# 0xPARC/plonkathon

Measured on NVIDIA H100. Metric: plonk_proofs_per_s_2^20_gates, higher is better.
Workload: dtype u256 (BN254 Fr/Fq integers, 8x32-bit Montgomery limbs)

## Files before the change

### include/plonk_b200.h

```cpp
#ifndef PLONK_B200_H
#define PLONK_B200_H
#include <stddef.h>
#include <stdint.h>

#ifdef __cplusplus
extern "C" {
#endif

typedef struct pb200_ctx pb200_ctx;
typedef struct pb200_srs pb200_srs;
typedef struct pb200_prover pb200_prover;
typedef struct pb200_transcript pb200_transcript;

const char* pb200_last_error(void);
const char* pb200_version(void);
int pb200_ctx_create(int device, void* cuda_stream, pb200_ctx** out);
void pb200_ctx_destroy(pb200_ctx* ctx);
int pb200_ctx_sync(pb200_ctx* ctx);
uint64_t pb200_ctx_launches(pb200_ctx* ctx);
int pb200_ctx_timing(pb200_ctx* ctx, int enable);
int pb200_ctx_timing_read(pb200_ctx* ctx, int category, double* total_ms, uint64_t* count);
void* pb200_ctx_stream(pb200_ctx* ctx);

int pb200_fr_to_mont(pb200_ctx* ctx, const void* d_in, void* d_out, uint64_t n);
// ... 5 lines not shown
int pb200_fr_ntt(pb200_ctx* ctx, const void* d_in, void* d_out, unsigned log_n, int inverse);
int pb200_fr_ntt_host(pb200_ctx* ctx, const uint8_t* h_in, uint8_t* h_out, unsigned log_n, int inverse);

int pb200_fr_ntt_decimated(pb200_ctx* ctx, const void* d_in, void* d_out, unsigned log_m, int inverse, uint64_t stride,
                           uint64_t offset);

int pb200_fr_coset_extend(pb200_ctx* ctx, const void* d_in, void* d_out, unsigned log_n, const uint8_t* h_offset);
int pb200_fr_coset_extend_host(pb200_ctx* ctx, const uint8_t* h_in, uint8_t* h_out, unsigned log_n,
                               const uint8_t* h_offset);
int pb200_fr_coset_to_coeffs(pb200_ctx* ctx, const void* d_in, void* d_out, unsigned log_n, const uint8_t* h_offset);
int pb200_fr_coset_to_coeffs_host(pb200_ctx* ctx, const uint8_t* h_in, uint8_t* h_out, unsigned log_n,
                                  const uint8_t* h_offset);
int pb200_fr_barycentric_eval(pb200_ctx* ctx, const void* d_vals, unsigned log_n, const uint8_t* h_x, uint8_t* h_out);
int pb200_fr_barycentric_eval_host(pb200_ctx* ctx, const uint8_t* h_vals, unsigned log_n, const uint8_t* h_x,
                                   uint8_t* h_out);

int pb200_g1_msm(pb200_ctx* ctx, const void* d_points, const void* d_scalars, uint64_t n, uint8_t* h_out_xy,
                 int* is_identity);
int pb200_g1_msm_host(pb200_ctx* ctx, const uint8_t* h_points, const uint8_t* h_scalars, uint64_t n,
                      uint8_t* h_out_xy, int* is_identity);

int pb200_srs_create(pb200_ctx* ctx, const uint8_t* h_points, uint64_t n, int precompute, pb200_srs** out);
int pb200_srs_generate(pb200_ctx* ctx, const uint8_t* h_tau, uint64_t n, int precompute, pb200_srs** out);
int pb200_srs_generate_lagrange(pb200_ctx* ctx, const uint8_t* h_tau, uint64_t n, int precompute, pb200_srs** out);
int pb200_srs_export(pb200_ctx* ctx, pb200_srs* srs, uint8_t* h_points, uint64_t first, uint64_t count);
void pb200_srs_destroy(pb200_srs* srs);
uint64_t pb200_srs_size(pb200_srs* srs);
int pb200_srs_commit_lagrange(pb200_ctx* ctx, pb200_srs* srs, const void* d_values, unsigned log_n,
                              uint8_t* h_out_xy, int* is_identity);
int pb200_srs_commit_lagrange_host(pb200_ctx* ctx, pb200_srs* srs, const uint8_t* h_values, unsigned log_n,
                                   uint8_t* h_out_xy, int* is_identity);
int pb200_srs_commit_coeffs(pb200_ctx* ctx, pb200_srs* srs, const void* d_coeffs, uint64_t m, int coeffs_montgomery,
                            uint8_t* h_out_xy, int* is_identity);
int pb200_srs_commit_coeffs_host(pb200_ctx* ctx, pb200_srs* srs, const uint8_t* h_coeffs, uint64_t m,
                                 uint8_t* h_out_xy, int* is_identity);

int pb200_prover_create(pb200_ctx* ctx, pb200_srs* srs, unsigned log_n, const uint8_t* const* h_pk,
                        pb200_prover** out);
int pb200_prover_create_custom(pb200_ctx* ctx, pb200_srs* srs, unsigned log_n, const uint8_t* const* h_pk,
                               unsigned n_custom, const uint8_t* h_exps, const uint8_t* const* h_custom,
                               pb200_prover** out);
void pb200_prover_destroy(pb200_prover* p);
int pb200_prover_prove(pb200_prover* p, const uint8_t* h_A, const uint8_t* h_B, const uint8_t* h_C,
                       const uint8_t* h_public, uint64_t n_public, uint8_t* h_proof768);
int pb200_prover_prove_device(pb200_prover* p, const void* d_A, const void* d_B, const void* d_C,
                              const uint8_t* h_public, uint64_t n_public, uint8_t* h_proof768);
int pb200_prover_round1(pb200_prover* p, const uint8_t* h_A, const uint8_t* h_B, const uint8_t* h_C,
                        const uint8_t* h_public, uint64_t n_public, uint8_t* h_abc_xy );
int pb200_prover_round2(pb200_prover* p, const uint8_t* beta, const uint8_t* gamma, uint8_t* h_z_xy);
int pb200_prover_round3(pb200_prover* p, const uint8_t* alpha, const uint8_t* fft_cofactor,
                        uint8_t* h_t_xy );
int pb200_prover_round4(pb200_prover* p, const uint8_t* zeta, uint8_t* h_evals );
int pb200_prover_round5(pb200_prover* p, const uint8_t* v, uint8_t* h_w_xy );

int pb200_prover_read_vector(pb200_prover* p, int which, void* d_out);
int pb200_prover_set_zk(pb200_prover* p, int enable, const uint8_t* h_blinders);
int pb200_prover_serialize(pb200_prover* p, uint8_t* h_proof768);

int pb200_prover_set_lookup(pb200_prover* p, const uint8_t* h_qk, const uint8_t* h_t1, const uint8_t* h_t2,
                            const uint8_t* h_t3, uint64_t table_rows);
int pb200_prover_set_lookup_tagged(pb200_prover* p, const uint8_t* h_qk, const uint8_t* h_qtag, const uint8_t* h_t1,
                                   const uint8_t* h_t2, const uint8_t* h_t3, const uint8_t* h_t4, uint64_t table_rows);
int pb200_prover_round_lookup(pb200_prover* p, const uint8_t* eta, uint8_t* h_fh_xy );
int pb200_prover_round2_lookup(pb200_prover* p, const uint8_t* beta, const uint8_t* gamma, const uint8_t* delta,
                               const uint8_t* epsilon, uint8_t* h_zz2_xy );
int pb200_prover_round4_lookup(pb200_prover* p, const uint8_t* zeta, uint8_t* h_evals );
// ... 65 lines not shown
```

### plonkathon_b200/_lib.py

```python
from __future__ import annotations

import ctypes
import os
import threading

_HERE = os.path.dirname(os.path.abspath(__file__))
LIB_PATH = os.environ.get("PB200_LIB") or os.path.join(_HERE, "libplonk_b200.so")

c_u8p = ctypes.POINTER(ctypes.c_uint8)


class PlonkB200Error(RuntimeError):
    pass


def _load():
    if not os.path.exists(LIB_PATH):
        raise PlonkB200Error(
            "libplonk_b200.so is not built (%s); run `python -c 'import __graft_entry__ as g; g.build()'`"
            % LIB_PATH)
    lib = ctypes.CDLL(LIB_PATH)
    V, I, U, U64 = ctypes.c_void_p, ctypes.c_int, ctypes.c_uint, ctypes.c_uint64
    P = ctypes.POINTER
    sig = {
# ... 10 lines not shown
        "pb200_fr_from_mont": (I, [V, V, V, U64]),
        "pb200_fr_ntt": (I, [V, V, V, U, I]),
        "pb200_fr_ntt_host": (I, [V, V, V, U, I]),
        "pb200_fr_ntt_decimated": (I, [V, V, V, U, I, U64, U64]),
        "pb200_fr_ntt_sharded": (I, [V, V, V, U, I]),
        "pb200_fr_vec_op": (I, [V, I, V, V, V, V, U64, U64]),
        "pb200_prover_read_vector": (I, [V, I, V]),
        "pb200_comm_unique_id": (I, [V]),
        "pb200_comm_init": (I, [V, V, I, I]),
        "pb200_comm_info": (I, [V, P(I), P(I), P(U64), P(U64)]),
        "pb200_srs_commit_coeffs_sharded": (I, [V, V, V, U64, I, V, P(I)]),
        "pb200_prover_create_sharded": (I, [V, V, U, V, P(V)]),
        "pb200_srs_commit_partial": (I, [V, V, V, U64, U64, U, U, I, V]),
        "pb200_srs_bucket_count": (I, [V, P(U)]),
        "pb200_g1_join_bucket_shards_host": (I, [V, U, U, U, V, P(I)]),
        "pb200_fr_coset_extend": (I, [V, V, V, U, V]),
        "pb200_fr_coset_extend_host": (I, [V, V, V, U, V]),
        "pb200_fr_coset_to_coeffs": (I, [V, V, V, U, V]),
        "pb200_fr_coset_to_coeffs_host": (I, [V, V, V, U, V]),
        "pb200_fr_barycentric_eval": (I, [V, V, U, V, V]),
        "pb200_fr_barycentric_eval_host": (I, [V, V, U, V, V]),
        "pb200_g1_msm": (I, [V, V, V, U64, V, P(I)]),
        "pb200_g1_msm_host": (I, [V, V, V, U64, V, P(I)]),
        "pb200_srs_create": (I, [V, V, U64, I, P(V)]),
        "pb200_srs_generate": (I, [V, V, U64, I, P(V)]),
        "pb200_srs_generate_lagrange": (I, [V, V, U64, I, P(V)]),
        "pb200_srs_export": (I, [V, V, V, U64, U64]),
        "pb200_srs_destroy": (None, [V]),
        "pb200_srs_size": (U64, [V]),
        "pb200_srs_commit_lagrange": (I, [V, V, V, U, V, P(I)]),
        "pb200_srs_commit_lagrange_host": (I, [V, V, V, U, V, P(I)]),
        "pb200_srs_commit_coeffs_host": (I, [V, V, V, U64, V, P(I)]),
        "pb200_srs_commit_coeffs": (I, [V, V, V, U64, I, V, P(I)]),
        "pb200_prover_create": (I, [V, V, U, V, P(V)]),
        "pb200_prover_create_custom": (I, [V, V, U, V, U, V, V, P(V)]),
        "pb200_prover_create_custom_sharded": (I, [V, V, U, V, U, V, V, P(V)]),
        "pb200_prover_destroy": (None, [V]),
        "pb200_prover_prove": (I, [V, V, V, V, V, U64, V]),
        "pb200_prover_prove_device": (I, [V, V, V, V, V, U64, V]),
        "pb200_prover_round1": (I, [V, V, V, V, V, U64, V]),
        "pb200_prover_round2": (I, [V, V, V, V]),
        "pb200_prover_round3": (I, [V, V, V, V]),
        "pb200_prover_round4": (I, [V, V, V]),
        "pb200_prover_round5": (I, [V, V, V]),
        "pb200_prover_serialize": (I, [V, V]),
        "pb200_prover_set_zk": (I, [V, I, V]),
        "pb200_prover_set_zk_lookup": (I, [V, I, V]),
        "pb200_prover_set_lookup": (I, [V, V, V, V, V, U64]),
        "pb200_prover_set_lookup_tagged": (I, [V, V, V, V, V, V, V, U64]),
        "pb200_prover_round_lookup": (I, [V, V, V]),
        "pb200_prover_round2_lookup": (I, [V, V, V, V, V, V]),
        "pb200_prover_round4_lookup": (I, [V, V, V]),
        "pb200_prover_prove_lookup": (I, [V, V, V, V, V, U64, V]),
        "pb200_prover_serialize_lookup": (I, [V, V]),
        "pb200_prover_create_custom_next_row": (I, [V, V, U, V, U, V, V, P(V)]),
        "pb200_prover_round4_next_row": (I, [V, V, V]),
        "pb200_prover_prove_next_row": (I, [V, V, V, V, V, U64, V]),
        "pb200_prover_serialize_next_row": (I, [V, V]),
        "pb200_prover_set_shuffle": (I, [V, V, V]),
        "pb200_prover_round2_shuffle": (I, [V, V, V, V, V, V]),
        "pb200_prover_round4_shuffle": (I, [V, V, V]),
        "pb200_prover_round4_next_row_shuffle": (I, [V, V, V]),
        "pb200_prover_prove_shuffle": (I, [V, V, V, V, V, U64, V]),
        "pb200_prover_serialize_shuffle": (I, [V, V]),
        "pb200_prover_prove_next_row_shuffle": (I, [V, V, V, V, V, U64, V]),
        "pb200_prover_serialize_next_row_shuffle": (I, [V, V]),
# ... 76 lines not shown
```

### plonkathon_b200/csrc/capi.cu

```cuda
#include "../../include/plonk_b200.h"

#include <cstring>

#include "common.cuh"
#include "comm.cuh"
#include "msm_bucket.cuh"
#include "prover.cuh"
#include "pairing.cuh"
#include "transcript.cuh"

namespace pb200 {
void ntt_run(Context* ctx, const Fr* in, Fr* out, int log_n, bool inverse, uint64_t n_in, const Fr* in_scale,
             const Fr* out_scale);
void launch_powers(Context* ctx, Fr* out, uint64_t n, const Fr& base, const Fr& scale);
Fr fr_from_u64(uint64_t x);
void ntt_run_strided(Context* ctx, const Fr* in, Fr* out, int log_n, bool inverse, uint64_t n_in,
                     const Fr* in_scale, const Fr* out_scale, uint64_t in_mul, uint64_t in_add);
void ntt_sharded(Context* ctx, const Fr* const* in, Fr* const* out, int count, int log_n, bool inverse);
void fr_to_mont(Context* ctx, const Fr* in, Fr* out, uint64_t n);
void fr_from_mont(Context* ctx, const Fr* in, Fr* out, uint64_t n);
void fr_vec_op(Context* ctx, int op, const Fr* a, const Fr* b, const Fr& scalar_canonical, Fr* out, uint64_t n,
               uint64_t shift);
void barycentric_eval(Context* ctx, const Fr* d_vals, int log_n, const Fr& x_mont, Fr* h_out);
float bench_modmul(Context* ctx, int field, uint64_t threads, uint32_t iters);
// ... 358 lines not shown
  PB_API_BEGIN PB_ON_CTX(C(ctx));
  srs_export(C(ctx), reinterpret_cast<Srs*>(srs), h_points, first, count);
  PB_API_END
}
void pb200_srs_destroy(pb200_srs* srs) { srs_destroy(reinterpret_cast<Srs*>(srs)); }
uint64_t pb200_srs_size(pb200_srs* srs) { return srs_size(reinterpret_cast<Srs*>(srs)); }

int pb200_srs_commit_lagrange(pb200_ctx* ctx, pb200_srs* srs, const void* d_values, unsigned log_n, uint8_t* h_out_xy,
                              int* is_identity) {
  PB_API_BEGIN PB_ON_CTX(C(ctx));
  Context* c = C(ctx);
  uint64_t n = (uint64_t)1 << log_n;
  PB_CHECK(n <= srs_size(reinterpret_cast<Srs*>(srs)), "Not enough powers in setup");
  DevBuf coeffs(n * 32);
  ntt_run(c, (const Fr*)d_values, coeffs.as<Fr>(), (int)log_n, true, n, nullptr, nullptr);
  srs_msm(c, reinterpret_cast<Srs*>(srs), coeffs.as<Fr>(), n, false, h_out_xy, is_identity);
  PB_API_END
}
int pb200_srs_commit_lagrange_host(pb200_ctx* ctx, pb200_srs* srs, const uint8_t* h_values, unsigned log_n,
                                   uint8_t* h_out_xy, int* is_identity) {
  PB_API_BEGIN PB_ON_CTX(C(ctx));
  size_t bytes = ((size_t)1 << log_n) * 32;
  HostStage st(C(ctx), h_values, bytes, 0);
  int rc = pb200_srs_commit_lagrange(ctx, srs, st.in.p, log_n, h_out_xy, is_identity);
  if (rc) throw Error(g_err);
  PB_API_END
}
int pb200_srs_commit_coeffs(pb200_ctx* ctx, pb200_srs* srs, const void* d_coeffs, uint64_t m, int coeffs_montgomery,
                            uint8_t* h_out_xy, int* is_identity) {
  PB_API_BEGIN PB_ON_CTX(C(ctx));
  srs_msm(C(ctx), reinterpret_cast<Srs*>(srs), (const Fr*)d_coeffs, m, coeffs_montgomery != 0, h_out_xy, is_identity);
  PB_API_END
}

int pb200_prover_create(pb200_ctx* ctx, pb200_srs* srs, unsigned log_n, const uint8_t* const* h_pk,
                        pb200_prover** out) {
  return pb200_prover_create_custom(ctx, srs, log_n, h_pk, 0, nullptr, nullptr, out);
}
int pb200_prover_create_sharded(pb200_ctx* ctx, pb200_srs* srs, unsigned log_n, const uint8_t* const* h_pk,
                                pb200_prover** out) {
  return pb200_prover_create_custom_sharded(ctx, srs, log_n, h_pk, 0, nullptr, nullptr, out);
}
int pb200_prover_create_custom(pb200_ctx* ctx, pb200_srs* srs, unsigned log_n, const uint8_t* const* h_pk,
                               unsigned n_custom, const uint8_t* h_exps, const uint8_t* const* h_custom,
                               pb200_prover** out) {
  PB_API_BEGIN PB_ON_CTX(C(ctx));
  *out = reinterpret_cast<pb200_prover*>(prover_create(C(ctx), reinterpret_cast<Srs*>(srs), (int)log_n, h_pk,
                                                       (int)n_custom, h_exps, h_custom, false, 3));
  PB_API_END
}
int pb200_prover_create_custom_next_row(pb200_ctx* ctx, pb200_srs* srs, unsigned log_n, const uint8_t* const* h_pk,
                                        unsigned n_custom, const uint8_t* h_exps, const uint8_t* const* h_custom,
                                        pb200_prover** out) {
  PB_API_BEGIN PB_ON_CTX(C(ctx));
  *out = reinterpret_cast<pb200_prover*>(prover_create(C(ctx), reinterpret_cast<Srs*>(srs), (int)log_n, h_pk,
                                                       (int)n_custom, h_exps, h_custom, false, 6));
  PB_API_END
}
int pb200_prover_create_custom_sharded(pb200_ctx* ctx, pb200_srs* srs, unsigned log_n, const uint8_t* const* h_pk,
                                       unsigned n_custom, const uint8_t* h_exps, const uint8_t* const* h_custom,
                                       pb200_prover** out) {
  PB_API_BEGIN PB_ON_CTX(C(ctx));
  *out = reinterpret_cast<pb200_prover*>(prover_create(C(ctx), reinterpret_cast<Srs*>(srs), (int)log_n, h_pk,
                                                       (int)n_custom, h_exps, h_custom, true, 3));
  PB_API_END
}
// ... 386 lines not shown
```

### plonkathon_b200/csrc/host_selftest.cpp

```cpp
#include "field.cuh"
#include "curve.cuh"
#include "msm_digits.cuh"
#include "modinv.cuh"
#include "msm_bucket.cuh"
#include "msm_sort.cuh"
#include "ntt_shard.cuh"
#include <algorithm>
#include <vector>
#include <cstring>
using namespace pb200;

template <class F> static F ld(const uint32_t* p) { F r; memcpy(r.v, p, 32); return r; }
template <class F> static void st(uint32_t* p, const F& a) { memcpy(p, a.v, 32); }

extern "C" {
int hs_field_op(int field, int op, const uint32_t* a, const uint32_t* b, uint32_t* out) {
#define RUN(F)                                                   \
  {                                                              \
    F x = ld<F>(a), y = ld<F>(b), r;                             \
    switch (op) {                                                \
      case 0: r = fp_add(x, y); break;                           \
      case 1: r = fp_sub(x, y); break;                           \
      case 2: r = fp_mul(x, y); break;                           \
      case 3: r = fp_neg(x); break;                              \
// ... 269 lines not shown
      for (uint32_t t = 0; t < bin_nt; t++)
        bin_reserve(a, t, bin_nt, runs[t], sh_cnt.data(), sh_loc.data(), sh_base.data());
      for (uint32_t t = 0; t < bin_nt; t++) bin_stage(a, bx, k, t, bin_nt, sh_cnt.data(), sh_loc.data(), bin_stage_buf.data());
      for (uint32_t t = 0; t < bin_nt; t++)
        bin_copy_out(a, t, bin_nt, total, sh_loc.data(), sh_base.data(), bin_stage_buf.data());
    }
  {
    std::vector<uint32_t> sums(256);
    for (uint32_t t = 0; t < 256; t++) sums[t] = chunk_map_sum(a, t);
    uint32_t run = 0;
    for (uint32_t t = 0; t < 256; t++) { const uint32_t s = sums[t]; sums[t] = run; run += s; }
    for (uint32_t t = 0; t < 256; t++) chunk_map_write(a, t, sums[t], run);
  }
  const uint32_t grid = 3;
  SortChunk ch;
  for (uint32_t bx = 0; bx < grid; bx++)
    for (uint32_t c = bx; chunk_locate(a, c, ch); c += grid) {
      for (uint32_t t = 0; t < chunk_nt; t++) sort_zero(sh_cnt.data(), ch.nkeys, t, chunk_nt);
      for (uint32_t t = 0; t < chunk_nt; t++) chunk_hist(a, ch, t, chunk_nt, sh_cnt.data());
      for (uint32_t t = 0; t < chunk_nt; t++) chunk_flush(a, ch, t, chunk_nt, sh_cnt.data());
    }
  host_scan(counts.data(), g.nb, pad, off.data(), &counts[g.nb]);
  sorted.assign(off[g.nb] + 2, PB_MSM_PAD);
  a.sorted = sorted.data();
  for (uint32_t bx = grid; bx-- > 0;)
    for (uint32_t c = bx; chunk_locate(a, c, ch); c += grid) {
      for (uint32_t t = 0; t < chunk_nt; t++) sort_zero(sh_cnt.data(), ch.nkeys, t, chunk_nt);
      for (uint32_t t = 0; t < chunk_nt; t++) chunk_hist(a, ch, t, chunk_nt, sh_cnt.data());
      const uint32_t total = block_scan(ch.nkeys, chunk_nt);
      for (uint32_t t = 0; t < chunk_nt; t++)
        chunk_reserve(a, ch, t, chunk_nt, runs[t], sh_cnt.data(), sh_loc.data(), sh_base.data());
      for (uint32_t t = 0; t < chunk_nt; t++) chunk_stage(a, ch, t, chunk_nt, sh_cnt.data(), sh_loc.data(), chunk_stage_buf.data());
      for (uint32_t t = 0; t < chunk_nt; t++)
        chunk_copy_out(a, ch, t, chunk_nt, sh_loc.data(), sh_base.data(), chunk_stage_buf.data());
      if (total != ch.hi - ch.lo) abort();
    }
}

extern "C" {
int hs_msm_sort(const uint32_t* scalars, uint32_t n, uint32_t batch, uint32_t c, int fixed_base, uint32_t lo,
                uint32_t hi, uint32_t pad, uint32_t lb, uint32_t T, uint32_t spb, uint32_t bin_nt, uint32_t chunk_nt,
                uint32_t* counts_out, uint32_t* off_out, uint32_t* sorted_out, uint32_t cap) {
  if (!n || !batch || batch > 4 || (!fixed_base && batch != 1) || c < 1 || c > 16 || !T || !bin_nt || !chunk_nt)
    return -1;
  MsmGeom g;
  if (!msm_geom(n, batch, c, fixed_base, lo, hi, g)) return -1;
  if (lb == 0xffffffffu) lb = sort_default_lb(g.nb);
  if (((g.nb - 1) >> lb) >= PB_SORT_MAX_BINS || (1u << lb) > PB_SORT_MAX_BIN_KEYS) return -1;
  if (!spb) spb = PB_SORT_BIN_STAGE / g.W;
  std::vector<Fr> sc((size_t)batch * n);
  for (size_t i = 0; i < sc.size(); i++) sc[i] = ld<Fr>(scalars + 8 * i);
  std::vector<uint32_t> counts, off, sorted;
  host_msm_sort(g, sc, n, pad ? 1 : 0, lb, T, spb, bin_nt, chunk_nt, counts, off, sorted);
  if (off[g.nb] > cap) return -1;
  memcpy(counts_out, counts.data(), counts.size() * 4);
  memcpy(off_out, off.data(), off.size() * 4);
  memcpy(sorted_out, sorted.data(), (size_t)off[g.nb] * 4);
  return (int)g.nb;
}

int hs_msm_pipeline(const uint32_t* points, uint32_t n, const uint32_t* scalars, uint32_t batch, uint32_t c,
                    int fixed_base, uint32_t lo, uint32_t hi, uint32_t B, uint32_t g0, uint32_t* out, uint8_t* out_inf) {
  if (!n || !batch || batch > 4 || (!fixed_base && batch != 1) || c < 1 || c > 16 || B < 2 || B > PB_AFF_BMAX) return -1;
  if (g0 < 2 || (g0 & (g0 - 1))) return -1;
  MsmGeom g;
  if (!msm_geom(n, batch, c, fixed_base, lo, hi, g)) return -1;
  std::vector<G1Affine> tab(fixed_base ? (size_t)g.W * n : n);
  for (uint32_t i = 0; i < n; i++) {
    tab[i].x = fp_to_mont(ld<Fq>(points + 16 * i));
    tab[i].y = fp_to_mont(ld<Fq>(points + 16 * i + 8));
  }
  if (fixed_base)
    for (uint32_t w = 1; w < g.W; w++)
      for (uint32_t i = 0; i < n; i++) {
        G1XYZZ a;
        g1_double_affine(a, tab[(size_t)(w - 1) * n + i]);
        for (uint32_t k = 1; k < c; k++) g1_double(a);
        g1_to_affine(a, tab[(size_t)w * n + i]);
      }
  std::vector<Fr> sc((size_t)batch * n);
  for (size_t i = 0; i < sc.size(); i++) sc[i] = ld<Fr>(scalars + 8 * i);
  std::vector<uint32_t> counts, off, sorted;
  host_msm_sort(g, sc, n, 1, sort_default_lb(g.nb), PB_SORT_CHUNK, PB_SORT_BIN_STAGE / g.W, PB_SORT_BIN_THREADS,
                PB_SORT_CHUNK_THREADS, counts, off, sorted);
  const uint32_t maxc = counts[g.nb];
  const uint64_t positions = (uint64_t)n * g.W * batch + g.nb, s_bound = positions / 2;
  std::vector<G1Affine> pts(s_bound + 1);
  AffAcc a;
  a.table = tab.data();
  a.sorted = sorted.data();
  a.pts = pts.data();
  a.off = off.data();
  a.cnt = counts.data();
  a.max_cnt = counts.data() + g.nb;
  a.nbl = g.nb;
  a.B = B;
  Fq pref[PB_AFF_BMAX];
  uint32_t desc[PB_AFF_BMAX];
  int rounds = 0;
  for (uint32_t r = 0; r < 32; r++) {
    a.r = r;
    if (r > 0 && maxc > (1u << r)) rounds = r + 1;
    if (r == 0) rounds = 1;
    const uint64_t T = aff_round_threads(s_bound, B, r) + 40;
    for (uint64_t t = T; t-- > 0;) {
      if (r == 0) aff_round0_thread(a, t, pref, desc);
      else aff_round_thread(a, t, pref, desc);
    }
  }
  ReduceArgs ra;
  ra.pts = pts.data(); ra.off = off.data(); ra.cnt = counts.data(); ra.xb = nullptr;
  ra.sets = g.sets; ra.m = g.nloc; ra.g = g0;
  std::vector<SR> cur((size_t)g.sets * reduce_groups(ra.m, ra.g)), nxt;
  ra.out = cur.data();
  for (uint64_t t = 0; t < cur.size() + 3; t++) reduce_level0_thread(ra, t);
  uint32_t m = reduce_groups(ra.m, ra.g), log_G = 0;
  while ((1u << log_G) < g0) log_G++;
// ... 72 lines not shown
```

### plonkathon_b200/csrc/msm.cu

```cuda
#include <algorithm>
#include <cstring>

#include "common.cuh"
#include "comm.cuh"
#include "msm_bucket.cuh"
#include "msm_digits.cuh"
#include "msm_sort.cuh"

namespace pb200 {

__device__ __forceinline__ G1Affine ld_affine(const G1Affine* p) {
  const uint4* q = reinterpret_cast<const uint4*>(p);
  uint4 a = __ldg(q), b = __ldg(q + 1), c = __ldg(q + 2), d = __ldg(q + 3);
  G1Affine r;
  r.x.v[0] = a.x; r.x.v[1] = a.y; r.x.v[2] = a.z; r.x.v[3] = a.w;
  r.x.v[4] = b.x; r.x.v[5] = b.y; r.x.v[6] = b.z; r.x.v[7] = b.w;
  r.y.v[0] = c.x; r.y.v[1] = c.y; r.y.v[2] = c.z; r.y.v[3] = c.w;
  r.y.v[4] = d.x; r.y.v[5] = d.y; r.y.v[6] = d.z; r.y.v[7] = d.w;
  return r;
}

__device__ __forceinline__ uint32_t block_exclusive_scan(uint32_t v, uint32_t* sh, uint32_t* total) {
  const uint32_t lane = threadIdx.x & 31, wid = threadIdx.x >> 5, nw = blockDim.x >> 5;
  uint32_t x = v;
  for (int d = 1; d < 32; d <<= 1) {
    uint32_t y = __shfl_up_sync(0xffffffffu, x, d);
    if ((int)lane >= d) x += y;
  }
  if (lane == 31) sh[wid] = x;
  __syncthreads();
  if (wid == 0) {
    uint32_t w = lane < nw ? sh[lane] : 0;
    for (int d = 1; d < 32; d <<= 1) {
      uint32_t y = __shfl_up_sync(0xffffffffu, w, d);
      if ((int)lane >= d) w += y;
    }
    if (lane < nw) sh[lane] = w;
  }
  __syncthreads();
  uint32_t base = wid ? sh[wid - 1] : 0;
  *total = sh[nw - 1];
  __syncthreads();
  return base + x - v;
}

__global__ void __launch_bounds__(PB_SORT_BIN_THREADS) k_msm_bin_count(SortArgs a) {
  __shared__ uint32_t sh_cnt[PB_SORT_MAX_BINS];
  const uint32_t t = threadIdx.x, nt = blockDim.x;
  sort_zero(sh_cnt, a.nbins, t, nt);
  __syncthreads();
  bin_hist(a, blockIdx.x, blockIdx.y, t, nt, sh_cnt);
  __syncthreads();
  bin_flush(a, t, nt, sh_cnt);
}

__global__ void __launch_bounds__(PB_SORT_BIN_THREADS) k_msm_bin_scatter(SortArgs a) {
  __shared__ uint32_t sh_cnt[PB_SORT_MAX_BINS], sh_loc[PB_SORT_MAX_BINS], sh_base[PB_SORT_MAX_BINS], sh_scan[32];
  extern __shared__ SortEntry stage[];
  const uint32_t t = threadIdx.x, nt = blockDim.x;
  sort_zero(sh_cnt, a.nbins, t, nt);
  __syncthreads();
  bin_hist(a, blockIdx.x, blockIdx.y, t, nt, sh_cnt);
  __syncthreads();
  uint32_t total;
  const uint32_t run = block_exclusive_scan(scan_part_sum(sh_cnt, a.nbins, t, nt), sh_scan, &total);
  bin_reserve(a, t, nt, run, sh_cnt, sh_loc, sh_base);
  __syncthreads();
  bin_stage(a, blockIdx.x, blockIdx.y, t, nt, sh_cnt, sh_loc, stage);
  __syncthreads();
  bin_copy_out(a, t, nt, total, sh_loc, sh_base, stage);
}

__global__ void __launch_bounds__(PB_SORT_CHUNK_THREADS) k_msm_chunk_count(SortArgs a) {
  __shared__ uint32_t sh_cnt[PB_SORT_MAX_BIN_KEYS];
  const uint32_t t = threadIdx.x, nt = blockDim.x;
  SortChunk ch;
  for (uint32_t c = blockIdx.x; chunk_locate(a, c, ch); c += gridDim.x) {
    sort_zero(sh_cnt, ch.nkeys, t, nt);
    __syncthreads();
    chunk_hist(a, ch, t, nt, sh_cnt);
    __syncthreads();
    chunk_flush(a, ch, t, nt, sh_cnt);
    __syncthreads();
  }
}

__global__ void __launch_bounds__(PB_SORT_CHUNK_THREADS) k_msm_chunk_place(SortArgs a) {
  __shared__ uint32_t sh_cnt[PB_SORT_MAX_BIN_KEYS], sh_loc[PB_SORT_MAX_BIN_KEYS], sh_base[PB_SORT_MAX_BIN_KEYS],
      sh_scan[32];
  extern __shared__ uint32_t stage_vals[];
  const uint32_t t = threadIdx.x, nt = blockDim.x;
  SortChunk ch;
  for (uint32_t c = blockIdx.x; chunk_locate(a, c, ch); c += gridDim.x) {
    sort_zero(sh_cnt, ch.nkeys, t, nt);
    __syncthreads();
    chunk_hist(a, ch, t, nt, sh_cnt);
    __syncthreads();
    uint32_t total;
    const uint32_t run = block_exclusive_scan(scan_part_sum(sh_cnt, ch.nkeys, t, nt), sh_scan, &total);
    chunk_reserve(a, ch, t, nt, run, sh_cnt, sh_loc, sh_base);
    __syncthreads();
    chunk_stage(a, ch, t, nt, sh_cnt, sh_loc, stage_vals);
    __syncthreads();
    chunk_copy_out(a, ch, t, nt, sh_loc, sh_base, stage_vals);
    __syncthreads();
  }
}

#define PB_SCAN_TILE 2048

__global__ void __launch_bounds__(256) k_scan_tile_sums(const uint32_t* counts, uint32_t nb, uint32_t pad,
                                                        uint32_t* tile_sums, uint32_t* max_out) {
  __shared__ uint32_t sh[8];
  uint32_t base = blockIdx.x * PB_SCAN_TILE + threadIdx.x * 8;
  uint32_t s = 0, m = 0;
  for (int k = 0; k < 8; k++)
    if (base + k < nb) {
      uint32_t c = counts[base + k];
      m = max(m, c);
      s += (c + pad) & ~pad;
    }
  uint32_t total;
  block_exclusive_scan(s, sh, &total);
  if (threadIdx.x == 0) tile_sums[blockIdx.x] = total;
  if (max_out) {
    for (int d = 16; d > 0; d >>= 1) m = max(m, __shfl_xor_sync(0xffffffffu, m, d));
    if ((threadIdx.x & 31) == 0 && m) atomicMax(max_out, m);
  }
}

__global__ void __launch_bounds__(256) k_scan_tiles(uint32_t* tile_sums, uint32_t n_tiles, uint32_t* total_out) {
  __shared__ uint32_t sh[8];
  uint32_t per = (n_tiles + 255) / 256;
  uint32_t lo = threadIdx.x * per, hi = min(lo + per, n_tiles);
  uint32_t s = 0;
  for (uint32_t i = lo; i < hi; i++) s += tile_sums[i];
  uint32_t total;
// ... 418 lines not shown
    }
  } else {
    comm = nullptr;
  }
  if (bucket_hi > g.half) bucket_hi = g.half;
  PB_CHECK(bucket_lo < bucket_hi, "empty MSM bucket range");
  g.lo = bucket_lo;
  g.nloc = bucket_hi - bucket_lo;
  g.sets = fixed_base ? batch : g.W;
  g.nb = g.sets * g.nloc;
  PB_CHECK((fixed_base ? (uint64_t)g.W * point_stride : n) < (1ull << 31), "MSM too large for 31-bit point ids");
  ScalarBatch sb;
  for (uint32_t k = 0; k < 4; k++) sb.p[k] = k < batch ? scalars[k] : nullptr;

  static const bool use_xyzz = [] { const char* e = getenv("PB200_MSM_ACC"); return !(e && !strcmp(e, "affine")); }();
  const uint32_t pad = use_xyzz ? 0 : 1;
  DevBuf& sorted = ctx->scratch[2];
  DevBuf& counts = ctx->scratch[3];
  DevBuf& offsets = ctx->scratch[4];
  DevBuf& lvl_a = ctx->scratch[6];
  DevBuf& lvl_b = ctx->scratch[7];
  const uint64_t entries = n * g.W * batch;
  const uint64_t positions = entries + (pad ? g.nb : 0);
  PB_CHECK(positions < (1ull << 30), "MSM too large (n * windows * batch must stay below 2^30)");
  sorted.ensure(positions * 4);
  counts.ensure((size_t)g.nb * 4 + 16);
  offsets.ensure((size_t)(g.nb + 1) * 4);
  uint32_t* max_cnt = counts.as<uint32_t>() + g.nb;
  const uint32_t n_tiles = (g.nb + PB_SCAN_TILE - 1) / PB_SCAN_TILE;
  PB_CHECK(n_tiles <= 8192, "too many buckets for the scan");
  ctx->msm_aff[1].ensure((size_t)8192 * 4);
  uint32_t* tile_sums = ctx->msm_aff[1].as<uint32_t>();

  const uint32_t lb = sort_default_lb(g.nb);
  PB_CHECK((1u << lb) <= PB_SORT_MAX_BIN_KEYS, "too many buckets for the sort");
  DevBuf& binned = ctx->scratch[8];
  DevBuf& bin_tab = ctx->scratch[9];
  binned.ensure(entries * sizeof(SortEntry));
  bin_tab.ensure((size_t)3 * (PB_SORT_MAX_BINS + 1) * 4);
  SortArgs sa;
  sa.sb = sb;
  sa.n = n;
  sa.from_mont = scalars_mont ? 1 : 0;
  sa.g = g;
  sa.lb = lb;
  sa.nbins = ((g.nb - 1) >> lb) + 1;
  sa.T = PB_SORT_CHUNK;
  uint32_t* bin_cnt = bin_tab.as<uint32_t>();
  uint32_t* bin_off = bin_cnt + PB_SORT_MAX_BINS + 1;
  sa.bin_cnt = bin_cnt;
  sa.bin_off = bin_off;
  sa.binned = binned.as<SortEntry>();
  sa.chunk_first = bin_off + PB_SORT_MAX_BINS + 1;
  sa.counts = counts.as<uint32_t>();
  sa.offsets = offsets.as<uint32_t>();
  sa.sorted = sorted.as<uint32_t>();
  sa.spb = PB_SORT_BIN_STAGE / g.W;
  const dim3 bin_grid((unsigned)((n + sa.spb - 1) / sa.spb), batch);
  const uint64_t chunk_bound = entries / PB_SORT_CHUNK + sa.nbins;
  const uint32_t count_grid = (uint32_t)std::min<uint64_t>((uint64_t)ctx->sm_count * 4, chunk_bound);
  const uint32_t place_grid = (uint32_t)std::min<uint64_t>((uint64_t)ctx->sm_count * 2, chunk_bound);
  const size_t bin_stage_bytes = PB_SORT_BIN_STAGE * sizeof(SortEntry), chunk_stage_bytes = PB_SORT_CHUNK * 4;
  PB_CUDA(cudaFuncSetAttribute(k_msm_bin_scatter, cudaFuncAttributeMaxDynamicSharedMemorySize, (int)bin_stage_bytes));
  PB_CUDA(cudaFuncSetAttribute(k_msm_chunk_place, cudaFuncAttributeMaxDynamicSharedMemorySize, (int)chunk_stage_bytes));

  cudaStream_t st = ctx->stream;
  ctx->time_begin(2);
  PB_CUDA(cudaMemsetAsync(counts.p, 0, (size_t)g.nb * 4 + 16, st));
  PB_CUDA(cudaMemsetAsync(bin_cnt, 0, (size_t)sa.nbins * 4, st));
  if (pad) PB_CUDA(cudaMemsetAsync(sorted.p, 0xff, positions * 4, st));
  k_msm_bin_count<<<bin_grid, PB_SORT_BIN_THREADS, 0, st>>>(sa);
  k_scan_tile_sums<<<1, 256, 0, st>>>(bin_cnt, sa.nbins, 0, tile_sums, nullptr);
  k_scan_tiles<<<1, 256, 0, st>>>(tile_sums, 1, bin_off + sa.nbins);
  k_scan_apply<<<1, 256, 0, st>>>(bin_cnt, sa.nbins, 0, tile_sums, bin_off);
  k_msm_bin_scatter<<<bin_grid, PB_SORT_BIN_THREADS, bin_stage_bytes, st>>>(sa);
  k_msm_chunk_map<<<1, 256, 0, st>>>(sa);
  k_msm_chunk_count<<<count_grid, PB_SORT_CHUNK_THREADS, 0, st>>>(sa);
  k_scan_tile_sums<<<n_tiles, 256, 0, st>>>(counts.as<uint32_t>(), g.nb, pad, tile_sums, max_cnt);
  k_scan_tiles<<<1, 256, 0, st>>>(tile_sums, n_tiles, offsets.as<uint32_t>() + g.nb);
  k_scan_apply<<<n_tiles, 256, 0, st>>>(counts.as<uint32_t>(), g.nb, pad, tile_sums, offsets.as<uint32_t>());
  k_msm_chunk_place<<<place_grid, PB_SORT_CHUNK_THREADS, chunk_stage_bytes, st>>>(sa);
  ctx->time_end(2);
  ctx->launches += 11;

  ReduceArgs ra;
  ra.pts = nullptr; ra.off = offsets.as<uint32_t>(); ra.cnt = counts.as<uint32_t>(); ra.xb = nullptr;
  if (!use_xyzz) {
    const uint64_t s_bound = positions / 2;
    DevBuf& pts = ctx->msm_aff[0];
    pts.ensure(s_bound * sizeof(G1Affine));
    AffAcc a;
    a.table = points;
    a.sorted = sorted.as<uint32_t>();
    a.pts = pts.as<G1Affine>();
    a.off = offsets.as<uint32_t>();
    a.cnt = counts.as<uint32_t>();
    a.max_cnt = max_cnt;
    a.nbl = g.nb;
    uint64_t cap = fixed_base ? n * g.W : n;
    uint32_t max_rounds = 1;
    while (max_rounds < 32 && (1ull << max_rounds) < cap) max_rounds++;
    ctx->time_begin(0);
    for (uint32_t r = 0; r < std::min<uint32_t>(max_rounds, PB_AFF_GRID_ROUNDS); r++) {
      a.r = r;
// ... 323 lines not shown
```

### plonkathon_b200/csrc/msm_sort.cuh

```cuda
#pragma once
#include "msm_digits.cuh"

namespace pb200 {

#define PB_SORT_MAX_BINS 2048
#define PB_SORT_MAX_BIN_KEYS 2048
#define PB_SORT_BIN_THREADS 512
#define PB_SORT_BIN_STAGE 8192
#define PB_SORT_CHUNK_THREADS 512
#define PB_SORT_CHUNK 16384
static_assert(PB_SORT_MAX_BINS <= 256 * 8, "k_msm_chunk_map and the bin scan take one block of 256 x 8 bins");

struct alignas(8) SortEntry {
  uint32_t key, val;
};

struct SortArgs {
  ScalarBatch sb;
  uint64_t n;
  int from_mont;
  MsmGeom g;
  uint32_t spb;
  uint32_t lb;
  uint32_t nbins;
  uint32_t T;
  uint32_t* bin_cnt;
  const uint32_t* bin_off;
  SortEntry* binned;
  uint32_t* chunk_first;
  uint32_t* counts;
  const uint32_t* offsets;
  uint32_t* sorted;
};

PB_HD uint32_t sort_default_lb(uint32_t nb) {
  uint32_t lb = 0;
  while (((nb - 1) >> lb) >= PB_SORT_MAX_BINS) lb++;
  return lb;
}

PB_HD uint32_t sort_add(uint32_t* p, uint32_t v) {
#if defined(__CUDA_ARCH__)
  return atomicAdd(p, v);
#else
  const uint32_t o = *p;
  *p = o + v;
  return o;
#endif
}

PB_HD void sort_zero(uint32_t* sh, uint32_t len, uint32_t t, uint32_t nt) {
  for (uint32_t b = t; b < len; b += nt) sh[b] = 0;
}

PB_HD uint32_t scan_part_sum(const uint32_t* sh, uint32_t len, uint32_t t, uint32_t nt) {
  const uint32_t per = (len + nt - 1) / nt;
  uint32_t s = 0;
  for (uint32_t b = t * per; b < t * per + per && b < len; b++) s += sh[b];
  return s;
}

template <class F>
PB_HD void sort_walk(const SortArgs& a, uint32_t bx, uint32_t k, uint32_t t, uint32_t nt, F f) {
  const uint64_t end = (uint64_t)(bx + 1) * a.spb < a.n ? (uint64_t)(bx + 1) * a.spb : a.n;
  for (uint64_t i = (uint64_t)bx * a.spb + t; i < end; i += nt) {
    DigitWalk dw(a.sb.p[k], i, a.from_mont);
    for (uint32_t w = 0; w < a.g.W; w++) {
      uint32_t neg, d = dw.next(w, a.g, neg);
      if (!d) continue;
      const uint32_t key = msm_bucket_key(a.g, k, w, d);
// ... 76 lines not shown
  return true;
}

PB_HD void chunk_hist(const SortArgs& a, const SortChunk& ch, uint32_t t, uint32_t nt, uint32_t* sh_cnt) {
  for (uint32_t i = ch.lo + t; i < ch.hi; i += nt) sort_add(&sh_cnt[a.binned[i].key - ch.key0], 1u);
}

PB_HD void chunk_flush(const SortArgs& a, const SortChunk& ch, uint32_t t, uint32_t nt, const uint32_t* sh_cnt) {
  for (uint32_t l = t; l < ch.nkeys; l += nt)
    if (sh_cnt[l]) sort_add(&a.counts[ch.key0 + l], sh_cnt[l]);
}

PB_HD void chunk_reserve(const SortArgs& a, const SortChunk& ch, uint32_t t, uint32_t nt, uint32_t run,
                         uint32_t* sh_cnt, uint32_t* sh_loc, uint32_t* sh_base) {
  const uint32_t per = (ch.nkeys + nt - 1) / nt;
  for (uint32_t l = t * per; l < t * per + per && l < ch.nkeys; l++) {
    const uint32_t c = sh_cnt[l];
    sh_loc[l] = run;
    run += c;
    if (c) sh_base[l] = a.offsets[ch.key0 + l] + sort_add(&a.counts[ch.key0 + l], c);
    sh_cnt[l] = 0;
  }
}

PB_HD void chunk_stage(const SortArgs& a, const SortChunk& ch, uint32_t t, uint32_t nt, uint32_t* sh_cnt,
                       const uint32_t* sh_loc, uint32_t* stage) {
  for (uint32_t i = ch.lo + t; i < ch.hi; i += nt) {
    const SortEntry e = a.binned[i];
    const uint32_t l = e.key - ch.key0;
    stage[sh_loc[l] + sort_add(&sh_cnt[l], 1u)] = e.val;
  }
}

PB_HD void chunk_copy_out(const SortArgs& a, const SortChunk& ch, uint32_t t, uint32_t nt, const uint32_t* sh_loc,
                          const uint32_t* sh_base, const uint32_t* stage) {
  for (uint32_t p = t; p < ch.hi - ch.lo; p += nt) {
    uint32_t lo = 0, hi = ch.nkeys;
    while (lo < hi) {
      const uint32_t m = (lo + hi) >> 1;
      if (sh_loc[m] > p) hi = m; else lo = m + 1;
    }
    a.sorted[sh_base[lo - 1] + p - sh_loc[lo - 1]] = stage[p];
  }
}

}
```

Before: 25.04.

## Retune MSM sort: larger chunks, adaptive bin width, warp-per-key copy-out, batch commit API

New measurement: 25.06 (median of 6 runs). Within noise of the previous version (+0.1%).

```diff
diff --git a/include/plonk_b200.h b/include/plonk_b200.h
--- a/include/plonk_b200.h
+++ b/include/plonk_b200.h
@@ -61,6 +61,8 @@
                                    uint8_t* h_out_xy, int* is_identity);
 int pb200_srs_commit_coeffs(pb200_ctx* ctx, pb200_srs* srs, const void* d_coeffs, uint64_t m, int coeffs_montgomery,
                             uint8_t* h_out_xy, int* is_identity);
+int pb200_srs_commit_coeffs_batch(pb200_ctx* ctx, pb200_srs* srs, const void* const* d_coeffs, unsigned batch,
+                                  uint64_t m, int coeffs_montgomery, uint8_t* h_out_xy, int* is_identity);
 int pb200_srs_commit_coeffs_host(pb200_ctx* ctx, pb200_srs* srs, const uint8_t* h_coeffs, uint64_t m,
                                  uint8_t* h_out_xy, int* is_identity);
 
diff --git a/plonkathon_b200/_lib.py b/plonkathon_b200/_lib.py
--- a/plonkathon_b200/_lib.py
+++ b/plonkathon_b200/_lib.py
@@ -66,6 +66,7 @@
         "pb200_srs_commit_lagrange_host": (I, [V, V, V, U, V, P(I)]),
         "pb200_srs_commit_coeffs_host": (I, [V, V, V, U64, V, P(I)]),
         "pb200_srs_commit_coeffs": (I, [V, V, V, U64, I, V, P(I)]),
+        "pb200_srs_commit_coeffs_batch": (I, [V, V, P(V), U, U64, I, V, P(I)]),
         "pb200_prover_create": (I, [V, V, U, V, P(V)]),
         "pb200_prover_create_custom": (I, [V, V, U, V, U, V, V, P(V)]),
         "pb200_prover_create_custom_sharded": (I, [V, V, U, V, U, V, V, P(V)]),
diff --git a/plonkathon_b200/csrc/capi.cu b/plonkathon_b200/csrc/capi.cu
--- a/plonkathon_b200/csrc/capi.cu
+++ b/plonkathon_b200/csrc/capi.cu
@@ -414,6 +414,14 @@
   srs_msm(C(ctx), reinterpret_cast<Srs*>(srs), (const Fr*)d_coeffs, m, coeffs_montgomery != 0, h_out_xy, is_identity);
   PB_API_END
 }
+int pb200_srs_commit_coeffs_batch(pb200_ctx* ctx, pb200_srs* srs, const void* const* d_coeffs, unsigned batch,
+                                  uint64_t m, int coeffs_montgomery, uint8_t* h_out_xy, int* is_identity) {
+  PB_API_BEGIN PB_ON_CTX(C(ctx));
+  PB_CHECK(batch >= 1 && batch <= 4, "batch must be 1..4");
+  srs_msm_batch(C(ctx), reinterpret_cast<Srs*>(srs), reinterpret_cast<const Fr* const*>(d_coeffs), batch, m,
+                coeffs_montgomery != 0, h_out_xy, is_identity);
+  PB_API_END
+}
 
 int pb200_prover_create(pb200_ctx* ctx, pb200_srs* srs, unsigned log_n, const uint8_t* const* h_pk,
                         pb200_prover** out) {
diff --git a/plonkathon_b200/csrc/host_selftest.cpp b/plonkathon_b200/csrc/host_selftest.cpp
--- a/plonkathon_b200/csrc/host_selftest.cpp
+++ b/plonkathon_b200/csrc/host_selftest.cpp
@@ -325,7 +325,7 @@
         chunk_reserve(a, ch, t, chunk_nt, runs[t], sh_cnt.data(), sh_loc.data(), sh_base.data());
       for (uint32_t t = 0; t < chunk_nt; t++) chunk_stage(a, ch, t, chunk_nt, sh_cnt.data(), sh_loc.data(), chunk_stage_buf.data());
       for (uint32_t t = 0; t < chunk_nt; t++)
-        chunk_copy_out(a, ch, t, chunk_nt, sh_loc.data(), sh_base.data(), chunk_stage_buf.data());
+        chunk_copy_out(a, ch, t, chunk_nt, total, sh_loc.data(), sh_base.data(), chunk_stage_buf.data());
       if (total != ch.hi - ch.lo) abort();
     }
 }
@@ -334,11 +334,11 @@
 int hs_msm_sort(const uint32_t* scalars, uint32_t n, uint32_t batch, uint32_t c, int fixed_base, uint32_t lo,
                 uint32_t hi, uint32_t pad, uint32_t lb, uint32_t T, uint32_t spb, uint32_t bin_nt, uint32_t chunk_nt,
                 uint32_t* counts_out, uint32_t* off_out, uint32_t* sorted_out, uint32_t cap) {
-  if (!n || !batch || batch > 4 || (!fixed_base && batch != 1) || c < 1 || c > 16 || !T || !bin_nt || !chunk_nt)
+  if (!n || !batch || batch > 4 || (!fixed_base && batch != 1) || c < 1 || c > 21 || !T || !bin_nt || !chunk_nt)
     return -1;
   MsmGeom g;
   if (!msm_geom(n, batch, c, fixed_base, lo, hi, g)) return -1;
-  if (lb == 0xffffffffu) lb = sort_default_lb(g.nb);
+  if (lb == 0xffffffffu) lb = sort_pick_lb(g.nb, (uint64_t)n * g.W * batch, T);
   if (((g.nb - 1) >> lb) >= PB_SORT_MAX_BINS || (1u << lb) > PB_SORT_MAX_BIN_KEYS) return -1;
   if (!spb) spb = PB_SORT_BIN_STAGE / g.W;
   std::vector<Fr> sc((size_t)batch * n);
@@ -374,8 +374,8 @@
   std::vector<Fr> sc((size_t)batch * n);
   for (size_t i = 0; i < sc.size(); i++) sc[i] = ld<Fr>(scalars + 8 * i);
   std::vector<uint32_t> counts, off, sorted;
-  host_msm_sort(g, sc, n, 1, sort_default_lb(g.nb), PB_SORT_CHUNK, PB_SORT_BIN_STAGE / g.W, PB_SORT_BIN_THREADS,
-                PB_SORT_CHUNK_THREADS, counts, off, sorted);
+  host_msm_sort(g, sc, n, 1, sort_pick_lb(g.nb, (uint64_t)n * g.W * batch, PB_SORT_CHUNK), PB_SORT_CHUNK,
+                PB_SORT_BIN_STAGE / g.W, PB_SORT_BIN_THREADS, PB_SORT_CHUNK_THREADS, counts, off, sorted);
   const uint32_t maxc = counts[g.nb];
   const uint64_t positions = (uint64_t)n * g.W * batch + g.nb, s_bound = positions / 2;
   std::vector<G1Affine> pts(s_bound + 1);
diff --git a/plonkathon_b200/csrc/msm.cu b/plonkathon_b200/csrc/msm.cu
--- a/plonkathon_b200/csrc/msm.cu
+++ b/plonkathon_b200/csrc/msm.cu
@@ -44,7 +44,7 @@
   return base + x - v;
 }
 
-__global__ void __launch_bounds__(PB_SORT_BIN_THREADS) k_msm_bin_count(SortArgs a) {
+__global__ void __launch_bounds__(PB_SORT_BIN_THREADS / 2) k_msm_bin_count(SortArgs a) {
   __shared__ uint32_t sh_cnt[PB_SORT_MAX_BINS];
   const uint32_t t = threadIdx.x, nt = blockDim.x;
   sort_zero(sh_cnt, a.nbins, t, nt);
@@ -102,7 +102,7 @@
     __syncthreads();
     chunk_stage(a, ch, t, nt, sh_cnt, sh_loc, stage_vals);
     __syncthreads();
-    chunk_copy_out(a, ch, t, nt, sh_loc, sh_base, stage_vals);
+    chunk_copy_out(a, ch, t, nt, total, sh_loc, sh_base, stage_vals);
     __syncthreads();
   }
 }
@@ -587,7 +587,7 @@
   ctx->msm_aff[1].ensure((size_t)8192 * 4);
   uint32_t* tile_sums = ctx->msm_aff[1].as<uint32_t>();
 
-  const uint32_t lb = sort_default_lb(g.nb);
+  const uint32_t lb = sort_pick_lb(g.nb, entries, PB_SORT_CHUNK);
   PB_CHECK((1u << lb) <= PB_SORT_MAX_BIN_KEYS, "too many buckets for the sort");
   DevBuf& binned = ctx->scratch[8];
   DevBuf& bin_tab = ctx->scratch[9];
@@ -614,7 +614,7 @@
   const dim3 bin_grid((unsigned)((n + sa.spb - 1) / sa.spb), batch);
   const uint64_t chunk_bound = entries / PB_SORT_CHUNK + sa.nbins;
   const uint32_t count_grid = (uint32_t)std::min<uint64_t>((uint64_t)ctx->sm_count * 4, chunk_bound);
-  const uint32_t place_grid = (uint32_t)std::min<uint64_t>((uint64_t)ctx->sm_count * 2, chunk_bound);
+  const uint32_t place_grid = (uint32_t)std::min<uint64_t>((uint64_t)ctx->sm_count, chunk_bound);
   const size_t bin_stage_bytes = PB_SORT_BIN_STAGE * sizeof(SortEntry), chunk_stage_bytes = PB_SORT_CHUNK * 4;
   PB_CUDA(cudaFuncSetAttribute(k_msm_bin_scatter, cudaFuncAttributeMaxDynamicSharedMemorySize, (int)bin_stage_bytes));
   PB_CUDA(cudaFuncSetAttribute(k_msm_chunk_place, cudaFuncAttributeMaxDynamicSharedMemorySize, (int)chunk_stage_bytes));
@@ -624,7 +624,7 @@
   PB_CUDA(cudaMemsetAsync(counts.p, 0, (size_t)g.nb * 4 + 16, st));
   PB_CUDA(cudaMemsetAsync(bin_cnt, 0, (size_t)sa.nbins * 4, st));
   if (pad) PB_CUDA(cudaMemsetAsync(sorted.p, 0xff, positions * 4, st));
-  k_msm_bin_count<<<bin_grid, PB_SORT_BIN_THREADS, 0, st>>>(sa);
+  k_msm_bin_count<<<bin_grid, PB_SORT_BIN_THREADS / 2, 0, st>>>(sa);
   k_scan_tile_sums<<<1, 256, 0, st>>>(bin_cnt, sa.nbins, 0, tile_sums, nullptr);
   k_scan_tiles<<<1, 256, 0, st>>>(tile_sums, 1, bin_off + sa.nbins);
   k_scan_apply<<<1, 256, 0, st>>>(bin_cnt, sa.nbins, 0, tile_sums, bin_off);
diff --git a/plonkathon_b200/csrc/msm_sort.cuh b/plonkathon_b200/csrc/msm_sort.cuh
--- a/plonkathon_b200/csrc/msm_sort.cuh
+++ b/plonkathon_b200/csrc/msm_sort.cuh
@@ -5,10 +5,10 @@
 
 #define PB_SORT_MAX_BINS 2048
 #define PB_SORT_MAX_BIN_KEYS 2048
-#define PB_SORT_BIN_THREADS 512
-#define PB_SORT_BIN_STAGE 8192
-#define PB_SORT_CHUNK_THREADS 512
-#define PB_SORT_CHUNK 16384
+#define PB_SORT_BIN_THREADS 1024
+#define PB_SORT_BIN_STAGE 16384
+#define PB_SORT_CHUNK_THREADS 1024
+#define PB_SORT_CHUNK 32768
 static_assert(PB_SORT_MAX_BINS <= 256 * 8, "k_msm_chunk_map and the bin scan take one block of 256 x 8 bins");
 
 struct alignas(8) SortEntry {
@@ -36,6 +36,12 @@
 PB_HD uint32_t sort_default_lb(uint32_t nb) {
   uint32_t lb = 0;
   while (((nb - 1) >> lb) >= PB_SORT_MAX_BINS) lb++;
+  return lb;
+}
+
+PB_HD uint32_t sort_pick_lb(uint32_t nb, uint64_t entries, uint32_t T) {
+  uint32_t lb = sort_default_lb(nb);
+  while ((2u << lb) <= PB_SORT_MAX_BIN_KEYS && (entries << (lb + 1)) <= (uint64_t)T * nb) lb++;
   return lb;
 }
 
@@ -178,15 +184,13 @@
   }
 }
 
-PB_HD void chunk_copy_out(const SortArgs& a, const SortChunk& ch, uint32_t t, uint32_t nt, const uint32_t* sh_loc,
-                          const uint32_t* sh_base, const uint32_t* stage) {
-  for (uint32_t p = t; p < ch.hi - ch.lo; p += nt) {
-    uint32_t lo = 0, hi = ch.nkeys;
-    while (lo < hi) {
-      const uint32_t m = (lo + hi) >> 1;
-      if (sh_loc[m] > p) hi = m; else lo = m + 1;
-    }
-    a.sorted[sh_base[lo - 1] + p - sh_loc[lo - 1]] = stage[p];
+PB_HD void chunk_copy_out(const SortArgs& a, const SortChunk& ch, uint32_t t, uint32_t nt, uint32_t total,
+                          const uint32_t* sh_loc, const uint32_t* sh_base, const uint32_t* stage) {
+  const uint32_t lane = t & 31, grp = t >> 5, ngrp = (nt + 31) >> 5;
+  const uint32_t gsz = nt - (grp << 5) < 32 ? nt - (grp << 5) : 32;
+  for (uint32_t l = grp; l < ch.nkeys; l += ngrp) {
+    const uint32_t s = sh_loc[l], e = l + 1 < ch.nkeys ? sh_loc[l + 1] : total;
+    for (uint32_t p = s + lane; p < e; p += gsz) a.sorted[sh_base[l] + p - s] = stage[p];
   }
 }
 
```
